# ftl/sdrainer

Measured on AMD Instinct MI355X. Metric: IQ MSamples/s through FFT+peak+envelope, higher is better.
Workload: dtype f64

## Files before the change

### sdrainer_amd/csrc/bank.h

```cpp
#pragma once
#include <hip/hip_runtime.h>

#include <algorithm>
#include <atomic>
#include <chrono>
#include <cmath>
#include <cstdio>
#include <cstdlib>
#include <cstring>
#include <memory>
#include <mutex>
#include <string>
#include <thread>
#include <vector>

#include "../../include/sdrainer_hip.h"
#include "host/delivery.h"
#include "host/frequency_mapping.h"
#include "sdr_device.h"

namespace sdrcapi {

inline thread_local std::string g_last_error;

// ... 72 lines not shown
    hipEvent_t done[sdr::K_COUNT] = {};
    void release()
    {
        psd.release();
        tap.release();
        tapw.release();
        tap_used.release();
        fft_ctr.release();
        fft_scratch.release();
        win_mean.release();
        cum_part.release();
        recs.release();
        raw_bits.release();
        bits.release();
        edges.release();
        edge_counts.release();
        tr_values.release();
        tr_raw.release();
        tr_deb.release();
        slots_before.release();
        cum_out.release();
        dev_peaks.release();
        peak_counts.release();
        for (auto &e : done) {
            if (e)
                (void)hipEventDestroy(e);
            e = nullptr;
        }
    }
};


enum Parts { PART_SPECTRA = 1, PART_LISTEN = 2, PART_ALL = 3 };

struct CursorPack {
    sdr::BatchCursor c[RING];
};

}

struct sdr_bank {
    template <class T>
    using DevBuf = sdrcapi::DevBuf<T>;
    using BatchSet = sdrcapi::BatchSet;
    static constexpr int N_STAGES = sdrcapi::N_STAGES, GRAPH_PHASES = sdrcapi::GRAPH_PHASES, N_GRAPHS = sdrcapi::N_GRAPHS, RING = sdrcapi::RING;

    sdr_config cfg{};
    sdr::Switches sw;
    int logn = 0;
    int hop = 0;
    int device = 0;
    hipStream_t stream[N_STAGES] = {};
    bool own_stream[N_STAGES] = {};

    int max_chunks = 0;
    int text_cap = 2048;
    int edge_cap = 0;
    int bit_words = 0;

    DevBuf<fft64::cplx> tw;
    DevBuf<unsigned char> db_tab;
    DevBuf<int32_t> tap_bins;
    DevBuf<float> window;
    bool windowed = false;
    DevBuf<float> spectrum_row;
    std::vector<BatchSet> set;
    DevBuf<sdr::BandState> band_state;
    DevBuf<sdr::ListenerSlot> slots;
    DevBuf<uint16_t> morse;
    DevBuf<uint32_t> text;
    DevBuf<uint32_t> text_frames;
    DevBuf<uint32_t> edge_pos;
    DevBuf<float> carry[2];

    std::vector<sdr::BandState> h_band_state;
    std::vector<sdr::ListenerSlot> h_slots;
    std::vector<int> n_slots;
    std::vector<int64_t> center_frequency;
    int carry_cur = 0;
    int cum_count = 0;
    int64_t total_frames = 0;
    int64_t batch_index = 0;
    int last_set = 0, last_frames = 0, last_chunks = 0, last_count0 = 0;
    int last_carry_in = 0;
    int edge_width = 0;
    int find_peaks = 1;
    bool failed = false;
    DevBuf<sdr::DropCounters> drops;
    DevBuf<sdr::BatchCursor> cursors;
    hipGraph_t graph[GRAPH_PHASES][N_GRAPHS] = {};
    hipGraphExec_t graph_exec[GRAPH_PHASES][N_GRAPHS] = {};
    hipGraphNode_t graph_cursor_node[GRAPH_PHASES] = {};
    hipEvent_t phase_done[GRAPH_PHASES][N_GRAPHS] = {};
    int64_t graph_base = 0;
    int64_t graph_replays = 0;
    bool graph_ready = false;
    int graph_frames = 0, graph_slots = 0;
    sdr::InFormat graph_fmt = sdr::InFormat::F32;
    uint64_t attach_gen = 0, graph_attach_gen = 0;
    bool graph_results_on = false;
    int graph_find_peaks = 0;
    bool defer_listen = false, listen_pending = false;
    struct PendingListen {
        int set = 0, frames = 0;
        int64_t first_frame = 0, batch = 0;
    } pend;
// ... 89 lines not shown
```

### sdrainer_amd/csrc/capi_bank.hip

```cpp
#include "bank.h"
#include "twiddles.h"

using namespace sdrcapi;

namespace sdr {
int set_error(int code, const char *msg) { return fail(code, msg); }
}

namespace sdrcapi {
std::unique_ptr<host::DeliveryBackend> make_results_backend(sdr_bank *b);

void resolve_profile(sdr_bank *b)
{
    for (auto &p : b->pending) {
        float ms = 0.f;
        if (hipEventElapsedTime(&ms, p.second.first, p.second.second) == hipSuccess) {
            b->prof_ms[p.first] += ms;
            b->prof_n[p.first] += 1;
        }
        (void)hipEventDestroy(p.second.first);
        (void)hipEventDestroy(p.second.second);
    }
    b->pending.clear();
}

int sync_bank(sdr_bank *b)
{
    HIP_TRY(hipSetDevice(b->device));
    {
        const int frc = flush_late_attached(b);
        if (frc)
            return frc;
    }
    for (int s = 0; s < N_STAGES; s++)
        HIP_TRY(hipStreamSynchronize(b->stream[s]));
    b->slots_put = false;
    resolve_profile(b);
    return SDR_OK;
}

int check_band(sdr_bank *b, int band)
{
    if (!b)
        return fail(SDR_ERR_BAD_ARG, "null bank");
    if (band < 0 || band >= b->cfg.n_bands)
        return fail(SDR_ERR_BAD_ARG, "band out of range");
    return SDR_OK;
}

int check_listener(sdr_bank *b, int band, int lid)
{
    int rc = check_band(b, band);
    if (rc)
        return rc;
    if (lid < 0 || lid >= b->n_slots[band])
        return fail(SDR_ERR_BAD_ARG, "listener id out of range");
    return SDR_OK;
}


hipError_t alloc_set(sdr_bank *b, BatchSet &S)
{
    const sdr_config &c = b->cfg;
    const size_t B = (size_t)c.n_bands, F = (size_t)c.max_batch_frames, L = (size_t)c.max_listeners, N = (size_t)c.block_size;
    hipError_t e = hipSuccess;
#define SET_ALLOC(buf, count)            \
    do {                                 \
        if (e == hipSuccess)             \
            e = (buf).alloc(count);      \
    } while (0)
    SET_ALLOC(S.psd, B * F * N);
    SET_ALLOC(S.tap, B * F * std::max<size_t>(L, 1));
    if (b->logn == 14) {
        SET_ALLOC(S.tapw, B * F * 4 * std::max<size_t>(L, 1));
        if (e == hipSuccess)
            e = S.tap_used.alloc(B * std::max<size_t>(L, 1), 0xff);
        SET_ALLOC(S.fft_ctr, B * 2);
    }
    SET_ALLOC(S.fft_scratch, B * (size_t)sdr::fft2p_group_frames(b->sw, c.block_size, c.n_bands, c.max_batch_frames) * N);
    SET_ALLOC(S.win_mean, B * F * 10);
    SET_ALLOC(S.recs, B * F);
    SET_ALLOC(S.raw_bits, B * L * (size_t)b->bit_words);
    SET_ALLOC(S.bits, B * L * (size_t)b->bit_words);
    SET_ALLOC(S.edges, B * L * (size_t)b->edge_cap);
    SET_ALLOC(S.edge_counts, B * L);
    if (c.trace) {
        SET_ALLOC(S.tr_values, B * F * L);
        SET_ALLOC(S.tr_raw, B * F * L);
        SET_ALLOC(S.tr_deb, B * F * L);
        SET_ALLOC(S.slots_before, B * L);
// ... 150 lines not shown
            return fail(SDR_ERR_HIP, "twiddle / table upload failed");
        }
    }
    b->res_backend = make_results_backend(b);
    b->results.reset(new host::Delivery(b->res_backend.get(), RING, GRAPH_PHASES * RING));
    b->set.reserve((size_t)RING + (size_t)GRAPH_PHASES * RING);
    b->set.resize(RING);
    for (int r = 0; r < RING; r++) {
        const hipError_t se = alloc_set(b, b->set[r]);
        if (se != hipSuccess) {
            sdr_destroy(b);
            return fail(SDR_ERR_HIP, std::string("allocating a batch buffer set: ") + hipGetErrorString(se));
        }
    }
    ALLOC(b->band_state, B);
    ALLOC(b->drops, 1);
    ALLOC(b->cursors, GRAPH_PHASES * RING);
    ALLOC(b->spectrum_row, (size_t)N);
    ALLOC(b->tap_bins, B * std::max<size_t>(L, 1));
    {
        std::vector<int32_t> free_bins(B * std::max<size_t>(L, 1), -1);
        hipError_t he = hipMemcpy(b->tap_bins.p, free_bins.data(), free_bins.size() * sizeof(int32_t), hipMemcpyHostToDevice);
        if (he != hipSuccess) {
            sdr_destroy(b);
            return fail(SDR_ERR_HIP, "tap table upload failed");
        }
    }
    ALLOC(b->slots, B * L);
    ALLOC(b->morse, cw::kMorseTableSize);
    ALLOC(b->text, B * L * (size_t)b->text_cap);
    ALLOC(b->text_frames, B * L * (size_t)b->text_cap);
    ALLOC(b->edge_pos, B * L * (size_t)cfg->max_batch_frames);
    ALLOC(b->carry[0], B * N);
    ALLOC(b->carry[1], B * N);
#undef ALLOC

    std::vector<uint16_t> h_morse(cw::kMorseTableSize);
    cw::build_morse_table(h_morse.data());
    hipError_t e = hipMemcpy(b->morse.p, h_morse.data(), sizeof(uint16_t) * cw::kMorseTableSize, hipMemcpyHostToDevice);
    b->h_band_state.assign(B, sdr::BandState{});
    for (auto &s : b->h_band_state)
        s.peak_threshold = cfg->peak_threshold;
    if (e == hipSuccess)
        e = hipMemcpy(b->band_state.p, b->h_band_state.data(), sizeof(sdr::BandState) * B, hipMemcpyHostToDevice);
    if (e != hipSuccess) {
        sdr_destroy(b);
        return fail(SDR_ERR_HIP, "state upload failed");
    }
    b->h_slots.assign(B * L, sdr::ListenerSlot{});
    b->n_slots.assign(B, 0);
    b->center_frequency.assign(B, 0);
    b->staged.assign(B, sdr::StreamStage{N, b->hop, 0, 0});
    b->staged_kind.assign(B, 0);
    *out = b;
    return SDR_OK;
}

int sdr_destroy(sdr_bank *b)
{
    if (!b)
        return SDR_OK;
    (void)hipSetDevice(b->device);
    for (int s = 0; s < N_STAGES; s++)
        (void)hipStreamSynchronize(b->stream[s]);
    resolve_profile(b);
    drop_graphs(b);
    if (b->slots_put_ev)
        (void)hipEventDestroy(b->slots_put_ev);
    for (auto &ph : b->phase_done)
        for (auto &ev : ph)
            if (ev)
                (void)hipEventDestroy(ev);
    b->tw.release();
    b->drops.release();
    b->cursors.release();
    b->db_tab.release();
    b->tap_bins.release();
    b->window.release();
    b->spectrum_row.release();
    for (auto &S : b->set)
        S.release();
    if (b->results)
        for (int i = 0; i < b->results->n_sets(); i++) {
            host::ResultSet &rs = b->results->set(i);
            if (rs.block)
                (void)hipHostFree(rs.block);
            if (rs.ev_listen)
                (void)hipEventDestroy(static_cast<hipEvent_t>(rs.ev_listen));
            if (rs.ev_peaks)
                (void)hipEventDestroy(static_cast<hipEvent_t>(rs.ev_peaks));
        }
    b->band_state.release();
    b->slots.release();
    b->morse.release();
    b->text.release();
    b->text_frames.release();
    b->edge_pos.release();
    b->carry[0].release();
    b->carry[1].release();
    for (int s = 0; s < N_STAGES; s++)
        if (b->own_stream[s] && b->stream[s])
            (void)hipStreamDestroy(b->stream[s]);
    if (b->copy_stream) {
        (void)hipStreamSynchronize(b->copy_stream);
        (void)hipStreamDestroy(b->copy_stream);
    }
    for (auto &st : b->stage) {
        if (st.h_f32)
            (void)hipHostFree(st.h_f32);
        if (st.h_raw)
            (void)hipHostFree(st.h_raw);
        st.d_f32.release();
        st.d_raw.release();
        if (st.uploaded)
            (void)hipEventDestroy(st.uploaded);
        if (st.consumed)
            (void)hipEventDestroy(st.consumed);
    }
    delete b;
    return SDR_OK;
}

int sdr_set_stream(sdr_bank *b, void *hip_stream)
{
    if (!b)
        return fail(SDR_ERR_BAD_ARG, "null bank");
    int rc = sync_bank(b);
    if (rc)
        return rc;
    for (int s = 1; s < N_STAGES; s++)
        if (!b->own_stream[s])
            b->stream[s] = reinterpret_cast<hipStream_t>(hip_stream);
    b->stream[S_FFT] = reinterpret_cast<hipStream_t>(hip_stream);
    return SDR_OK;
}

int sdr_sync(sdr_bank *b)
{
    if (!b)
        return fail(SDR_ERR_BAD_ARG, "null bank");
    return sync_bank(b);
}

int sdr_attach(sdr_bank *b, int band, int bin, int *listener_id)
{
    int rc = check_band(b, band);
    if (rc)
        return rc;
    const sdr_config &c = b->cfg;
    if (bin < 0 || bin >= c.block_size)
        return fail(SDR_ERR_BAD_ARG, "bin out of range");
    int lid = -1;
    for (int i = 0; i < b->n_slots[band]; i++)
        if (!b->h_slots[(size_t)band * c.max_listeners + i].active) {
            lid = i;
            break;
        }
    if (lid < 0) {
        if (b->n_slots[band] >= c.max_listeners)
            return fail(SDR_ERR_NO_SLOT, "listener pool exhausted");
        lid = b->n_slots[band]++;
    }
    sdr::ListenerSlot &s = b->h_slots[(size_t)band * c.max_listeners + lid];
    memset(&s, 0, sizeof s);
    s.active = 1;
    s.bin = bin;
    cw::debouncer_init(s.deb, c.signal_debounce);
    cw::decoder_init(s.dec, c.sample_rate, sdr::effective_hop(c.hop, c.block_size));
    cw::decoder_reset(s.dec);
    s.start_frame = s.tapped_from = (uint32_t)b->total_frames;
    rc = sync_bank(b);
    if (rc)
        return rc;
    HIP_TRY(hipMemcpy(b->slots.p + (size_t)band * c.max_listeners + lid, &s, sizeof s, hipMemcpyHostToDevice));
    const int32_t tap_bin = bin;
    HIP_TRY(hipMemcpy(b->tap_bins.p + (size_t)band * c.max_listeners + lid, &tap_bin, sizeof tap_bin, hipMemcpyHostToDevice));
    b->attach_gen++;
    if (listener_id)
        *listener_id = lid;
    return SDR_OK;
}

int sdr_detach(sdr_bank *b, int band, int lid)
{
    int rc = check_listener(b, band, lid);
    if (rc)
        return rc;
// ... 209 lines not shown
```

### sdrainer_amd/csrc/capi_process.hip

```cpp
#include <string>

#include "bank.h"

using namespace sdrcapi;

namespace sdrcapi {

constexpr int PUT_SLOTS = 16, PUT_BINS = 128;
struct SlotPack {
    int32_t n;
    int32_t index[PUT_SLOTS];
    sdr::ListenerSlot slot[PUT_SLOTS];
};
struct BinPack {
    int32_t n;
    int32_t index[PUT_BINS], bin[PUT_BINS];
};
__global__ void k_put_slots(sdr::ListenerSlot *slots, SlotPack p)
{
    constexpr int W = sizeof(sdr::ListenerSlot) / 4;
    static_assert(sizeof(sdr::ListenerSlot) % 4 == 0, "word copy");
    for (int i = threadIdx.x; i < p.n * W; i += blockDim.x)
        reinterpret_cast<uint32_t *>(slots + p.index[i / W])[i % W] = reinterpret_cast<const uint32_t *>(&p.slot[i / W])[i % W];
}
// ... 33 lines not shown
        HIP_TRY(hipGetLastError());
    }
    b->late_attached.clear();
    return SDR_OK;
}


int process_device_impl(sdr_bank *b, const void *iq_dev, int n_frames, size_t in_stride, sdr::InFormat fmt)
{
    if (b->failed)
        return fail(SDR_ERR_STATE, "an earlier process call failed half way; destroy the bank");
    if (b->graph_ready)
        return fail(SDR_ERR_STATE, "a graph is captured: process through sdr_graph_launch, or sdr_graph_release first");
    if (b->listen_pending)
        return fail(SDR_ERR_STATE, "the previous batch still waits for its listen half (sdr_process_listen)");
    const int rc = process_device_body(b, iq_dev, n_frames, in_stride, -1, -1, b->defer_listen ? PART_SPECTRA : PART_ALL, fmt);
    if (rc == SDR_ERR_HIP)
        b->failed = true;
    return rc;
}

int process_device_body(sdr_bank *b, const void *iq_dev, int n_frames, size_t in_stride, int capture_k, int capture_stage, int parts,
                        sdr::InFormat fmt)
{
    const bool cap = capture_k >= 0;
    const bool do_spectra = (parts & PART_SPECTRA) != 0, do_listen = (parts & PART_LISTEN) != 0;
    if (!do_spectra)
        n_frames = b->pend.frames;
    const sdr::BatchCursor *cur = cap ? b->cursors.p + capture_k : nullptr;
    const sdr_config &c = b->cfg;
    if (n_frames <= 0)
        return SDR_OK;
    struct DisarmOnExit {
        ~DisarmOnExit() { sdr::t_done_event = nullptr; }
    } disarm_on_exit;
    if (n_frames > c.max_batch_frames)
        return fail(SDR_ERR_BAD_ARG, "n_frames exceeds max_batch_frames");
    HIP_TRY(hipSetDevice(b->device));
    if (!cap) {
        const int frc = flush_late_attached(b);
        if (frc)
            return frc;
    }
    const int B = c.n_bands, N = c.block_size, stride = c.max_batch_frames;
    const sdr::NoiseGeom ng = b->noise_geom();
    const int si = cap ? RING + capture_k : do_spectra ? (int)(b->batch_index % RING) : b->pend.set;
    const int64_t first_frame = do_spectra ? b->total_frames : b->pend.first_frame;
    BatchSet &S = b->set[si];
    host::ResultSet &RS = b->results->set(si);
    int max_slots = 0;
    for (int i = 0; i < B; i++)
        max_slots = std::max(max_slots, b->n_slots[i]);
    const int count0 = b->cum_count;
    const sdr::BatchPlan P = sdr::plan_batch(b->sw, sdr::BatchGeometry{B, N, stride, b->max_chunks}, n_frames, count0, cap, max_slots, b->windowed);
    const int *plan = P.stream;
    const sdr::CumGeom cg{N, stride, n_frames, count0, b->max_chunks};
#define SDR_ON(k) (!cap || (capture_stage == G_THRESHOLDS ? (k) == sdr::K_THRESHOLDS : (plan[k] == capture_stage && (k) != sdr::K_THRESHOLDS)))
#if defined(SDR_DIAG)
#define SDR_LAUNCH(id, call) \
    do {                     \
        if (!(b->sw.diag_skip >> (id) & 1) && SDR_ON(id)) \
            HIP_TRY(call);   \
    } while (0)
#else
#define SDR_LAUNCH(id, call)  \
    do {                      \
        if (SDR_ON(id))       \
            HIP_TRY(call);    \
    } while (0)
#endif
    auto stream_of = [&](int k) { return b->stream[plan[k]]; };
    auto after = [&](int k, int dep) -> int {
        if (stream_of(k) != stream_of(dep) && !cap)
            HIP_TRY(hipStreamWaitEvent(stream_of(k), S.done[dep], 0));
        return SDR_OK;
    };
#define SDR_AFTER(k, dep)          \
    do {                           \
        int _rc = after((k), (dep)); \
        if (_rc)                   \
            return _rc;            \
    } while (0)
#define SDR_ARM(k) (sdr::t_done_event = cap ? nullptr : S.done[k])
#define SDR_DONE(k)                                                                                   \
    do {                                                                                              \
        if (sdr::t_done_event && !cap) {                                                              \
            sdr::t_done_event = nullptr;                                                              \
            HIP_TRY(hipEventRecord(S.done[k], stream_of(k)));                                         \
        }                                                                                             \
    } while (0)

    if (do_spectra) {
    if (b->results_on && !cap) {
        const int prc = b->results->park(si);
        if (prc)
            return prc;
    }
    {
        static const int launch_order[] = {sdr::K_WINDOW_MEANS, sdr::K_NOISE_STATS, sdr::K_THRESHOLDS, sdr::K_LISTEN_GATHER,
                                           sdr::K_LISTEN_DECODE, sdr::K_CUMULATE,   sdr::K_FIND_PEAKS};
        int last_on[N_STAGES];
        for (int &l : last_on)
            l = -1;
        for (int k : launch_order)
            last_on[plan[k]] = k;
        for (int st = 0; st < N_STAGES; st++) {
            const int k = last_on[st];
// ... 478 lines not shown
```

### sdrainer_amd/csrc/host/batch_plan.h

```cpp
#pragma once
#include <cstdint>
#include <cstdlib>
#include <cstring>

#include "../../../include/sdrainer_hip.h"

namespace sdr {

enum KernelId {
    K_FFT = 0, K_WINDOW_MEANS, K_NOISE_STATS, K_THRESHOLDS, K_LISTEN_GATHER, K_CUMULATE, K_FIND_PEAKS, K_LISTEN_DECODE,
    K_COUNT
};
enum Stage { S_FFT = 0, S_NOISE, S_LISTEN, S_PEAKS, N_STAGES };

constexpr int kR32MaxTap = 512;

struct Switches {
    bool noise_scan = true;
    int force_exact = 0;
    int fft_r32 = -1;
    int fft_fpw = 0;
    int cum_bound = -1;
    int refine_wide = -1;
    int var_mfma = -1;
    int wm_wpb = 0;
    int fft2p_group_mb = -1;
    bool no_overlap = false;
    bool graph_debug = false;
    int diag_skip = 0;
    int diag_plan[K_COUNT] = {-1, -1, -1, -1, -1, -1, -1, -1};
};

inline int tri_state(const char *e)
{
    if (!e)
        return -1;
    const int v = atoi(e);
    return v >= 0 ? (v != 0 ? 1 : 0) : -1;
}

inline Switches read_switches()
{
    Switches s;
    const char *e;
    if ((e = getenv("SDR_NOISE_PATH")))
        s.noise_scan = strcmp(e, "chains") != 0;
    if ((e = getenv("SDR_NOISE_FORCE_EXACT")))
        s.force_exact = atoi(e);
    if ((e = getenv("SDR_FFT_R32")))
        s.fft_r32 = atoi(e) ? 1 : 0;
    if ((e = getenv("SDR_FFT_FPW"))) {
        const int v = atoi(e);
        s.fft_fpw = v < 1 ? 1 : (v > 64 ? 64 : v);
    }
    s.cum_bound = tri_state(getenv("SDR_CUM_BOUND"));
    s.refine_wide = tri_state(getenv("SDR_REFINE_WIDE"));
    s.var_mfma = tri_state(getenv("SDR_VAR_MFMA"));
    if ((e = getenv("SDR_FFT2P_GROUP_MB")))
        s.fft2p_group_mb = atoi(e) >= 0 ? atoi(e) : -1;
    if ((e = getenv("SDR_WM_WPB")))
        s.wm_wpb = atoi(e) > 0 ? atoi(e) : 0;
    e = getenv("SDR_NO_OVERLAP");
    s.no_overlap = e && e[0] == '1';
    s.graph_debug = getenv("SDR_GRAPH_DEBUG") != nullptr;
#if defined(SDR_DIAG)
    if ((e = getenv("SDR_DIAG_SKIP")))
        s.diag_skip = atoi(e);
    if ((e = getenv("SDR_DIAG_PLAN")))
        for (int k = 0; k < K_COUNT && e[k] >= '0' && e[k] < '0' + N_STAGES; k++)
            s.diag_plan[k] = e[k] - '0';
#endif
    return s;
}

inline bool noise_scan_at(const Switches &sw, int n) { return sw.noise_scan && n <= 16384; }
inline bool var_mfma_at(const Switches &sw, int n, int n_frames)
{
    if (sw.var_mfma >= 0)
        return sw.var_mfma != 0;
    return n <= 16384 && n_frames < 4096;
}
inline bool may_use_matrix_pipe(const Switches &sw, int n) { return !noise_scan_at(sw, n) && (sw.var_mfma == 1 || (sw.var_mfma < 0 && n <= 16384)); }

struct FftChoice {
    bool r32 = false;
    int fpw = 0;
    bool wide_tap = false;
    bool two_phase = false;
    int group_frames = 0;
};

constexpr int kFft2pGroupMiB = 128;
inline int fft2p_group_frames(const Switches &sw, int n, int n_bands, int max_frames)
{
    if (n <= 16384 || n_bands <= 0 || max_frames <= 0)
        return 0;
    const int mib = sw.fft2p_group_mb >= 0 ? sw.fft2p_group_mb : kFft2pGroupMiB;
    const long per_frame = (long)n_bands * n * 16;
    const long f = mib == 0 ? max_frames : ((long)mib << 20) / per_frame;
    return (int)(f < 1 ? 1 : (f > max_frames ? max_frames : f));
}

inline FftChoice fft_choice(const Switches &sw, int n, int n_frames, int n_bands, int tap_n, bool windowed = false)
{
    FftChoice c;
    c.r32 = !windowed && n == 16384 && tap_n <= kR32MaxTap && (sw.fft_r32 == 1 || (sw.fft_r32 < 0 && (long)n_frames * n_bands >= 1024));
    c.fpw = sw.fft_fpw;
    c.wide_tap = c.r32 && tap_n > 0;
    c.two_phase = n > 16384;
    return c;
}

enum class Refine { NONE, NARROW, WIDE };

struct BatchGeometry {
    int n_bands, n, max_batch_frames, max_chunks;
};

struct BatchPlan {
    int stream[K_COUNT];
    FftChoice fft;
    bool noise_scan;
    int force_exact;
    bool var_mfma;
    int wm_wpb;
    bool bound;
    bool bound_done;
    int scan_parts;
    int n_slots;
    int n_chunks;
    int new_count;
    Refine refine;
};

inline BatchPlan plan_batch(const Switches &sw, const BatchGeometry &g, int n_frames, int count0, bool capturing, int max_slots,
                            bool windowed = false)
{
    BatchPlan p;
    const int plan[K_COUNT] = { S_FFT,         S_NOISE,  S_NOISE,  S_PEAKS,
                                S_LISTEN,   S_PEAKS,      S_PEAKS,   S_LISTEN};
    for (int k = 0; k < K_COUNT; k++)
        p.stream[k] = plan[k];
    if (!capturing && (long)g.n_bands * g.n <= 8192)
        p.stream[K_LISTEN_GATHER] = S_PEAKS;
    for (int k = 0; k < K_COUNT; k++)
        if (sw.diag_plan[k] >= 0)
            p.stream[k] = sw.diag_plan[k];

    p.fft = fft_choice(sw, g.n, n_frames, g.n_bands, max_slots, windowed);
    p.fft.group_frames = fft2p_group_frames(sw, g.n, g.n_bands, g.max_batch_frames);

    p.noise_scan = noise_scan_at(sw, g.n);
    p.force_exact = sw.force_exact;
    p.var_mfma = var_mfma_at(sw, g.n, n_frames);
    p.wm_wpb = sw.wm_wpb;

    p.bound = sw.cum_bound >= 0 ? sw.cum_bound != 0 : (double)n_frames * (double)g.n_bands * (double)g.n >= 64.0 * 1024.0 * 1024.0;
    p.bound_done = p.noise_scan && p.bound;

    p.n_chunks = (count0 + n_frames) / SDR_CUMULATION_SIZE;
    p.new_count = (count0 + n_frames) % SDR_CUMULATION_SIZE;
    p.n_slots = p.n_chunks + (p.new_count != 0 ? 1 : 0);
    if (capturing) {
        p.n_chunks = (SDR_CUMULATION_SIZE - 1 + n_frames) / SDR_CUMULATION_SIZE;
        p.n_slots = p.n_chunks + 1;
    }
    p.scan_parts = (long)p.n_slots * g.n_bands < 64 ? 2 : 1;

    const bool wide = sw.refine_wide >= 0 ? sw.refine_wide != 0 : (g.n >= 4096 && (long)p.n_chunks * g.n_bands >= 64);
    p.refine = !p.bound ? Refine::NONE : wide ? Refine::WIDE : Refine::NARROW;
    return p;
}

}
```

### sdrainer_amd/csrc/k_fft_psd.hip

```cpp
#include <hip/hip_runtime.h>

#include <algorithm>
#include <cstdlib>
#include <mutex>

#include "../../include/sdrainer_hip.h"
#include "cw_decoder.h"
#include "fft_f64.h"
#include "fft_r32.h"
#include "gomath.h"
#include "sc16.h"
#include "sdr_device.h"

#if !defined(SDR_FFT_WIN)
#define SDR_FFT_WIN 0
#endif
#if SDR_FFT_WIN
#define SDR_K_FFT_PSD k_fft_psd_win
#define SDR_K_FFT_PSD_SC16 k_fft_psd_sc16_win
#define SDR_WIN_PARAM , const float *__restrict__ win
#define SDR_WIN_ARG , win
#else
#define SDR_K_FFT_PSD k_fft_psd
#define SDR_K_FFT_PSD_SC16 k_fft_psd_sc16
// ... 896 lines not shown
        return hipGetLastError();
    }
    int fpw = fpw_asked > 0 ? fpw_asked : kDefaultFpw;
    while (fpw > 1 && (long)((n_frames + fpw - 1) / fpw) * n_bands < 256)
        fpw /= 2;
    if (fpw > 1)
        launch_kernel((SDR_K_FFT_PSD<LOGN, true>), dim3((n_frames + fpw - 1) / fpw, n_bands), dim3(PL::T), fft64::kLdsBytes<LOGN>, stream,
                           iq, cur, tw, psd, in_stride, frame_stride, out_stride, n_frames, fpw, tap.bins, tap.out, tap.n, tap.stride SDR_WIN_ARG);
    else
        launch_kernel((SDR_K_FFT_PSD<LOGN, false>), dim3(n_frames, n_bands), dim3(PL::T),
                           fft64::kLdsBytes<LOGN> + tap_lds + kPfSinkBytes, stream, iq, cur, tw, psd, in_stride,
                           frame_stride, out_stride, n_frames, 1, tap.bins, tap.out, tap.n, tap.stride SDR_WIN_ARG);
    return hipGetLastError();
    }
}

#if SDR_FFT_WIN
void window_layout(int logn, const float *w, float *out)
{
    switch (logn) {
    case 9: window_layout_t<9>(w, out); break;
    case 10: window_layout_t<10>(w, out); break;
    case 11: window_layout_t<11>(w, out); break;
    case 12: window_layout_t<12>(w, out); break;
    case 13: window_layout_t<13>(w, out); break;
    case 14: window_layout_t<14>(w, out); break;
    default:
        for (int i = 0; i < 1 << logn; i++)
            out[i] = w[i];
        break;
    }
}

hipError_t launch_fft_win(int logn, FftChoice fft, InFormat fmt, const void *iq, const BatchCursor *cur, const fft64::cplx *tw, float *psd,
                          int n_frames, int n_bands, size_t in_stride, int frame_stride, int out_stride, FftTap tap, hipStream_t stream)
{
    if (!tap.window || fft.r32 || fft.two_phase)
        return hipErrorInvalidValue;
#else
hipError_t launch_fft(int logn, FftChoice fft, InFormat fmt, const void *iq, const BatchCursor *cur, const fft64::cplx *tw, float *psd,
                      int n_frames, int n_bands, size_t in_stride, int frame_stride, int out_stride, FftTap tap, hipStream_t stream)
{
    if (fmt != InFormat::F32 && fmt != InFormat::SC16)
        return hipErrorInvalidValue;
    if (fft.two_phase)
        return launch_fft_2p(logn, fft, fmt, iq, cur, tw, psd, n_frames, n_bands, in_stride, frame_stride, out_stride, tap, stream);
    if (tap.window)
        return launch_fft_win(logn, fft, fmt, iq, cur, tw, psd, n_frames, n_bands, in_stride, frame_stride, out_stride, tap, stream);
    if (fft.r32) {
        if (logn != 14)
            return hipErrorInvalidValue;
        const fft64::cplx *tw32 = tw + fft64::Plan<14>::TW_TOTAL;
        if (fmt == InFormat::SC16)
            return launch_fft_r32_sc16(static_cast<const int16_t *>(iq), cur, tw32, psd, n_frames, n_bands, in_stride, frame_stride, out_stride, tap, stream);
        return launch_fft_r32(static_cast<const float *>(iq), cur, tw32, psd, n_frames, n_bands, in_stride, frame_stride, out_stride, tap, stream);
    }
#endif
    switch (logn) {
    case 9: return launch_fft_t<9>(fft.fpw, fmt, iq, cur, tw, psd, n_frames, n_bands, in_stride, frame_stride, out_stride, tap, stream);
    case 10: return launch_fft_t<10>(fft.fpw, fmt, iq, cur, tw, psd, n_frames, n_bands, in_stride, frame_stride, out_stride, tap, stream);
    case 11: return launch_fft_t<11>(fft.fpw, fmt, iq, cur, tw, psd, n_frames, n_bands, in_stride, frame_stride, out_stride, tap, stream);
    case 12: return launch_fft_t<12>(fft.fpw, fmt, iq, cur, tw, psd, n_frames, n_bands, in_stride, frame_stride, out_stride, tap, stream);
    case 13: return launch_fft_t<13>(fft.fpw, fmt, iq, cur, tw, psd, n_frames, n_bands, in_stride, frame_stride, out_stride, tap, stream);
    case 14: return launch_fft_t<14>(fft.fpw, fmt, iq, cur, tw, psd, n_frames, n_bands, in_stride, frame_stride, out_stride, tap, stream);
    default: return hipErrorInvalidValue;
    }
}
#if !SDR_FFT_WIN
hipError_t launch_fft(int logn, FftChoice fft, const float *iq, const BatchCursor *cur, const fft64::cplx *tw, float *psd, int n_frames,
                      int n_bands, size_t in_stride, int frame_stride, int out_stride, FftTap tap, hipStream_t stream)
{
    return launch_fft(logn, fft, InFormat::F32, iq, cur, tw, psd, n_frames, n_bands, in_stride, frame_stride, out_stride, tap, stream);
}

int twiddle_count(int logn)
{
    switch (logn) {
    case 9: return fft64::Plan<9>::TW_TOTAL;
    case 10: return fft64::Plan<10>::TW_TOTAL;
    case 11: return fft64::Plan<11>::TW_TOTAL;
    case 12: return fft64::Plan<12>::TW_TOTAL;
    case 13: return fft64::Plan<13>::TW_TOTAL;
    case 14: return fft64::Plan<14>::TW_TOTAL + r32_twiddle_count();
    case 15: return 1 << 14;
    case 16: return 1 << 15;
    default: return 0;
    }
}

void build_twiddles(int logn, const double *wre, const double *wim, fft64::cplx *out)
{
    switch (logn) {
    case 9: fft64::build_pass_twiddles<9>(wre, wim, out); break;
    case 10: fft64::build_pass_twiddles<10>(wre, wim, out); break;
    case 11: fft64::build_pass_twiddles<11>(wre, wim, out); break;
    case 12: fft64::build_pass_twiddles<12>(wre, wim, out); break;
    case 13: fft64::build_pass_twiddles<13>(wre, wim, out); break;
    case 14:
        fft64::build_pass_twiddles<14>(wre, wim, out);
        r32_build_twiddles(wre, wim, out + fft64::Plan<14>::TW_TOTAL);
        break;
    case 15:
    case 16:
        for (int i = 0; i < 1 << (logn - 1); i++)
            out[i] = fft64::cplx{wre[i], wim[i]};
        break;
    default: break;
    }
// ... 5 lines not shown
```

### sdrainer_amd/csrc/k_fft_r32.hip

```cpp
#include <hip/hip_runtime.h>

#include <algorithm>
#include <mutex>

#include "fft_r32.h"
#include "sdr_device.h"

#if !defined(SDR_R32_SC16)
#define SDR_R32_SC16 0
#endif
#if !defined(SDR_R32_HOP)
#define SDR_R32_HOP 0
#endif
#if SDR_R32_SC16
#include "sc16.h"
#define SDR_R32_IN int16_t
#else
#define SDR_R32_IN float
#endif
#if SDR_R32_HOP && SDR_R32_SC16
#define SDR_R32_KERNEL k_fft_r32_hop_sc16
#define SDR_R32_LAUNCH launch_fft_r32_hop_sc16
#elif SDR_R32_HOP
#define SDR_R32_KERNEL k_fft_r32_hop
// ... 437 lines not shown
        __syncthreads();
        SDR_R32_STAMP(st, RS_ROW);
        pf_point(PF_ROW);
        {
#pragma unroll
            for (int j = 0; j < N / 4 / T; j++)
                sv[j] = *reinterpret_cast<const u32x4 *>(smem + row_word(4 * (t + T * j)) * 4);
            const float *row = reinterpret_cast<const float *>(smem);
            const float tv = row[row_word(my_bin & (N - 1))];
            tapv = my_bin >= 0 ? tv : 0.0f;
            if (__builtin_amdgcn_readfirstlane(t) < n_tap && wide_b) {
                const rsrc_t wr = make_rsrc(wide_b + (size_t)frame * (4 * tap_stride), reg_tap ? (unsigned)tap_stride * 16u : 0u);
                u32x4 wv;
                wv.x = __float_as_uint(row[row_word((my_bin - 1) & (N - 1))]);
                wv.y = __float_as_uint(tv);
                wv.z = __float_as_uint(row[row_word((my_bin + 1) & (N - 1))]);
                wv.w = 0u;
                __builtin_amdgcn_raw_buffer_store_b128(wv, wr, t < n_tap ? (unsigned)t * 16u : 0x7ffffff0u, 0, 0);
            }
        }
        const unsigned after = __builtin_amdgcn_readfirstlane(claim_lds[0]);
        soft_arrive(soft + SOFT_ROW);
        SDR_R32_STAMP(st, RS_STORED);
#if defined(SDR_R32_PHASES)
        if (st.on && (threadIdx.x & 63) < RS_COUNT)
            g_r32_phases[threadIdx.x >> 6][threadIdx.x & 63] = st.v;
#endif
        prev = frame;
        frame = next;
        next = after;
        it++;
    }
    int t = tid;
    asm volatile("" : "+v"(t));
    flush_row(prev, t, 0, N / 4 / T);
    if (t == 0) {
        unsigned *const ctr = band_ctr();
        const unsigned done = __hip_atomic_fetch_add(ctr + 1, 1u, __ATOMIC_ACQ_REL, __HIP_MEMORY_SCOPE_AGENT);
        if (done == stash[2] - 1) {
            __hip_atomic_store(ctr, 0u, __ATOMIC_RELAXED, __HIP_MEMORY_SCOPE_AGENT);
            __hip_atomic_store(ctr + 1, 0u, __ATOMIC_RELAXED, __HIP_MEMORY_SCOPE_AGENT);
        }
    }
#endif
}

}

#if !SDR_R32_SC16 && !SDR_R32_HOP
int r32_twiddle_count() { return fft32::kTwTotal; }
void r32_build_twiddles(const double *wre, const double *wim, fft64::cplx *out) { fft32::build_twiddles(wre, wim, out); }
#endif

#if !defined(SDR_R32_RESERVE)
#define SDR_R32_RESERVE 0
#endif

hipError_t SDR_R32_LAUNCH(const SDR_R32_IN *iq, const BatchCursor *cur, const fft64::cplx *tw, float *psd, int n_frames, int n_bands,
                          size_t in_stride, int frame_stride, int out_stride, FftTap tap, hipStream_t stream)
{
    constexpr int kMaxDevices = 64;
    static std::once_flag setup_once[kMaxDevices];
    static hipError_t setup_err[kMaxDevices];
    static int cu_count[kMaxDevices];
    int dev = 0;
    hipError_t e = hipGetDevice(&dev);
    if (e != hipSuccess)
        return e;
    if (dev < 0 || dev >= kMaxDevices)
        return hipErrorInvalidDevice;
    std::call_once(setup_once[dev], [dev] {
        hipError_t se = hipFuncSetAttribute(reinterpret_cast<const void *>(&r32::SDR_R32_KERNEL), hipFuncAttributeMaxDynamicSharedMemorySize,
                                            r32::kLdsBytes);
        if (se == hipSuccess)
            se = hipDeviceGetAttribute(&cu_count[dev], hipDeviceAttributeMultiprocessorCount, dev);
        setup_err[dev] = se;
    });
    if (setup_err[dev] != hipSuccess)
        return setup_err[dev];
    if (n_frames <= 0 || n_bands <= 0)
        return hipSuccess;
    if (tap.n > fft32::T)
        return hipErrorInvalidValue;
    if (!tap.steal)
        return hipErrorInvalidValue;
    if (in_stride > 0xffffffffu)
        return hipErrorInvalidValue;
#if SDR_R32_HOP
    int shift = 0;
    while ((1 << shift) < frame_stride)
        shift++;
    if (frame_stride <= 0 || (1 << shift) != frame_stride || n_frames >= (1 << r32::kFrameBits))
        return hipErrorInvalidValue;
    const unsigned frames_and_shift = (unsigned)n_frames | (unsigned)shift << r32::kFrameBits;
#else
    if (frame_stride != fft32::N)
#if SDR_R32_SC16
        return launch_fft_r32_hop_sc16(iq, cur, tw, psd, n_frames, n_bands, in_stride, frame_stride, out_stride, tap, stream);
#else
        return launch_fft_r32_hop(iq, cur, tw, psd, n_frames, n_bands, in_stride, frame_stride, out_stride, tap, stream);
#endif
    const unsigned frames_and_shift = (unsigned)n_frames;
#endif
    const int cus = std::max(1, cu_count[dev] - SDR_R32_RESERVE);
    const int grid = std::min((cus + n_bands - 1) / n_bands, n_frames);
    launch_kernel(r32::SDR_R32_KERNEL, dim3(grid, n_bands), dim3(fft32::T), r32::kLdsBytes, stream, iq, cur, tw, psd, (unsigned)in_stride, out_stride,
                  frames_and_shift, tap.steal, tap.bins, tap.out, tap.n, tap.stride, tap.wide, tap.used);
    return hipGetLastError();
}

}
```

### sdrainer_amd/csrc/sdr_device.h

```cpp
#pragma once
#include <hip/hip_ext.h>
#include <hip/hip_runtime.h>

#include <cstdint>
#include <initializer_list>
#include <mutex>

#include "../../include/sdrainer_hip.h"
#include "cw_decoder.h"
#include "fft_f64.h"
#include "host/batch_plan.h"
#include "host/overlap.h"

namespace sdr {

struct BandState {
    float nf_ring[SDR_NOISE_WINDOW];
    float dev_ring[SDR_NOISE_WINDOW];
    float nf_sum, dev_sum;
    int32_t next;
    float peak_threshold;
};

struct ListenerSlot {
// ... 73 lines not shown
    if (done)
        hipExtLaunchKernelGGL(kernel, grid, block, lds_bytes, stream, nullptr, done, 0, args...);
    else
        hipLaunchKernelGGL(kernel, grid, block, lds_bytes, stream, args...);
}

struct LdsLimitOnce {
    static constexpr int kMaxDevices = 64;
    std::once_flag dev[kMaxDevices];
};
inline hipError_t raise_lds_limit_once(LdsLimitOnce &once, std::initializer_list<const void *> kernels, int bytes)
{
    int dev = 0;
    hipError_t e = hipGetDevice(&dev);
    if (e != hipSuccess)
        return e;
    if (dev < 0 || dev >= LdsLimitOnce::kMaxDevices)
        return hipErrorInvalidDevice;
    hipError_t attr_err = hipSuccess;
    std::call_once(once.dev[dev], [&] {
        for (const void *k : kernels) {
            const hipError_t ae = hipFuncSetAttribute(k, hipFuncAttributeMaxDynamicSharedMemorySize, bytes);
            if (ae != hipSuccess)
                attr_err = ae;
        }
    });
    return attr_err;
}

struct FftTap {
    const int32_t *bins;
    float *out;
    int n;
    int stride;
    float *wide = nullptr;
    int32_t *used = nullptr;
    uint32_t *steal = nullptr;
    fft64::cplx *scratch = nullptr;
    const float *window = nullptr;
};

hipError_t launch_fft(int logn, FftChoice fft, InFormat fmt, const void *iq, const BatchCursor *cur, const fft64::cplx *tw, float *psd,
                      int n_frames, int n_bands, size_t in_stride, int frame_stride, int out_stride, FftTap tap, hipStream_t stream);
hipError_t launch_fft(int logn, FftChoice fft, const float *iq, const BatchCursor *cur, const fft64::cplx *tw, float *psd, int n_frames,
                      int n_bands, size_t in_stride, int frame_stride, int out_stride, FftTap tap, hipStream_t stream);
hipError_t launch_fft_win(int logn, FftChoice fft, InFormat fmt, const void *iq, const BatchCursor *cur, const fft64::cplx *tw, float *psd,
                          int n_frames, int n_bands, size_t in_stride, int frame_stride, int out_stride, FftTap tap, hipStream_t stream);
void window_layout(int logn, const float *w, float *out);
hipError_t launch_fft_2p(int logn, FftChoice fft, InFormat fmt, const void *iq, const BatchCursor *cur, const fft64::cplx *tw, float *psd,
                         int n_frames, int n_bands, size_t in_stride, int frame_stride, int out_stride, FftTap tap, hipStream_t stream);
int twiddle_count(int logn);
void build_twiddles(int logn, const double *wre, const double *wim, fft64::cplx *out);
hipError_t launch_fft_r32(const float *iq, const BatchCursor *cur, const fft64::cplx *tw, float *psd, int n_frames, int n_bands,
                          size_t in_stride, int frame_stride, int out_stride, FftTap tap, hipStream_t stream);
hipError_t launch_fft_r32_sc16(const int16_t *iq, const BatchCursor *cur, const fft64::cplx *tw, float *psd, int n_frames, int n_bands,
                               size_t in_stride, int frame_stride, int out_stride, FftTap tap, hipStream_t stream);
hipError_t launch_fft_r32_hop(const float *iq, const BatchCursor *cur, const fft64::cplx *tw, float *psd, int n_frames, int n_bands,
                              size_t in_stride, int frame_stride, int out_stride, FftTap tap, hipStream_t stream);
hipError_t launch_fft_r32_hop_sc16(const int16_t *iq, const BatchCursor *cur, const fft64::cplx *tw, float *psd, int n_frames, int n_bands,
                                   size_t in_stride, int frame_stride, int out_stride, FftTap tap, hipStream_t stream);
int r32_twiddle_count();
void r32_build_twiddles(const double *wre, const double *wim, fft64::cplx *out);
hipError_t launch_window_means(const float *psd, double *win_mean, NoiseGeom g, int n_frames, int n_bands, int stride, int wpb_forced,
                               hipStream_t stream);
hipError_t launch_noise_stats(const float *psd, const double *win_mean, sdr_frame_rec *recs, NoiseGeom g, int n_frames,
                              int n_bands, int stride, bool mfma, hipStream_t stream);
hipError_t launch_mfma_order_probe(unsigned *mismatches, int order, hipStream_t stream);
hipError_t launch_thresholds(sdr_frame_rec *recs, BandState *st, int n_frames, int n_bands, int stride,
                             hipStream_t stream);
hipError_t launch_listen_gather(const float *tap, const float *psd, const sdr_frame_rec *recs, const ListenerSlot *slots, const void *db_tab,
                                uint64_t *raw_bits, float *tr_values, uint8_t *tr_raw, const BatchCursor *cur, ListenGeom g, int n_frames,
                                int n_slots, int n_bands, hipStream_t stream);
hipError_t launch_listen_decode(ListenerSlot *slots, const uint16_t *morse, const uint64_t *raw_bits,
                                uint64_t *deb_bits, uint32_t *text, uint32_t *text_frames, sdr_edge *edges,
                                uint32_t *edge_counts, uint8_t *tr_deb, DropCounters *drops, const BatchCursor *cur, ListenGeom g,
                                int n_frames, int n_bands, uint32_t *edge_pos, int pos_stride, hipStream_t stream);
hipError_t launch_listener_stop(ListenerSlot *slot, const uint16_t *morse, uint32_t *text, uint32_t *text_frames, int text_cap,
                                uint32_t frame, DropCounters *drops, hipStream_t stream);
hipError_t launch_set_debounce(ListenerSlot *slots, int n, int threshold, hipStream_t stream);
hipError_t launch_cumulate(const float *psd, const void *db_tab, float *carry0, float *carry1, int carry_in, float *cum_out,
                           const float *cum_part, const BatchCursor *cur, CumGeom g, int n_slots, int n_bands, bool bound, bool bound_done,
                           int parts, hipStream_t stream);
hipError_t launch_psd_scan(const float *psd, sdr_frame_rec *recs, float *cum_out, float *cum_part, const BatchCursor *cur, NoiseGeom ng,
                           CumGeom cg, int n_slots, int n_bands, bool do_bound, int parts, int force_exact, hipStream_t stream);
hipError_t launch_noise_exact_check(const float *psd_band, sdr_frame_rec *recs_band, NoiseGeom ng, int n_frames, unsigned *mismatches,
                                    hipStream_t stream);
hipError_t launch_spectrum_row(const float *psd_row, float *out, int n, hipStream_t stream);
hipError_t launch_pack_listen(ListenerSlot *slots, const sdr_edge *edges, const uint32_t *edge_counts, const uint32_t *text,
                              const uint32_t *text_frames, const DropCounters *drops, ResultsLayout lay, int n_slots, int n_bands, unsigned char *host,
                              hipStream_t stream);
hipError_t launch_pack_peaks(const DevPeak *peaks, const int *counts, const BatchCursor *cur, ResultsLayout lay, int find_peaks,
                             int n_frames, int n_chunks, int n_bands, unsigned char *host, hipStream_t stream);
__host__ __device__ inline int chunks_completed(int count0, int n_frames)
{
    const int first_len = SDR_CUMULATION_SIZE - count0;
    return n_frames >= first_len ? 1 + (n_frames - first_len) / SDR_CUMULATION_SIZE : 0;
}
hipError_t launch_unpack_be16(const uint8_t *raw, float *out, size_t n_values, hipStream_t stream);
hipError_t launch_unpack_sc16(const int16_t *raw, float *out, size_t n_values, hipStream_t stream);
hipError_t launch_find_peaks(float *cum, const float *psd, const void *db_tab, const float *carry0, const float *carry1, int carry_in,
                             const sdr_frame_rec *recs, DevPeak *peaks, int *counts, const BatchCursor *cur, PeakGeom g, int n_frames,
                             int n_chunks, int n_bands, Refine refine, FftTap tap, hipStream_t stream);
hipError_t launch_cumulation_row(const float *psd_band, const void *db_tab, const float *carry_in_band, float *row_out, CumGeom g, int slot,
                                 hipStream_t stream);

}
```

Before: 198,700.

## Reserve CUs for overlapping noise scan by capping r32 FFT grid size

```diff
diff --git a/sdrainer_amd/csrc/bank.h b/sdrainer_amd/csrc/bank.h
--- a/sdrainer_amd/csrc/bank.h
+++ b/sdrainer_amd/csrc/bank.h
@@ -148,6 +148,7 @@
     int device = 0;
     hipStream_t stream[N_STAGES] = {};
     bool own_stream[N_STAGES] = {};
+    bool fft_queue_alone = true;
 
     int max_chunks = 0;
     int text_cap = 2048;
diff --git a/sdrainer_amd/csrc/capi_bank.hip b/sdrainer_amd/csrc/capi_bank.hip
--- a/sdrainer_amd/csrc/capi_bank.hip
+++ b/sdrainer_amd/csrc/capi_bank.hip
@@ -36,6 +36,68 @@
         HIP_TRY(hipStreamSynchronize(b->stream[s]));
     b->slots_put = false;
     resolve_profile(b);
+    return SDR_OK;
+}
+
+constexpr int kProbeSpinUs = 300;
+__global__ void k_queue_probe_spin(unsigned ticks, unsigned *sink)
+{
+    const unsigned long long t0 = wall_clock64();
+    unsigned n = 0;
+    for (int i = 0; i < (1 << 20) && wall_clock64() - t0 < ticks; i++) {
+        __builtin_amdgcn_s_sleep(32);
+        n++;
+    }
+    if (n == 0xffffffffu)
+        *sink = n;
+}
+__global__ void k_queue_probe_nop() {}
+
+int probe_fft_queue(sdr_bank *b)
+{
+    b->fft_queue_alone = true;
+    if (b->cfg.block_size != 16384 || b->sw.no_overlap || b->sw.fft_reserve >= 0)
+        return SDR_OK;
+    HIP_TRY(hipSetDevice(b->device));
+    hipEvent_t spin_done = nullptr, nop_done[N_STAGES] = {};
+    auto cleanup = [&] {
+        if (spin_done)
+            (void)hipEventDestroy(spin_done);
+        for (hipEvent_t e : nop_done)
+            if (e)
+                (void)hipEventDestroy(e);
+    };
+    hipError_t e = hipEventCreateWithFlags(&spin_done, hipEventDisableTiming);
+    for (int s = 1; s < N_STAGES && e == hipSuccess; s++)
+        e = hipEventCreateWithFlags(&nop_done[s], hipEventDisableTiming);
+    for (int s = 0; s < N_STAGES && e == hipSuccess; s++) {
+        hipLaunchKernelGGL(k_queue_probe_nop, dim3(1), dim3(1), 0, b->stream[s]);
+        e = hipStreamSynchronize(b->stream[s]);
+    }
+    if (e == hipSuccess) {
+        hipLaunchKernelGGL(k_queue_probe_spin, dim3(1), dim3(1), 0, b->stream[S_FFT], (unsigned)kProbeSpinUs * 100u, reinterpret_cast<unsigned *>(b->drops.p));
+        e = hipEventRecord(spin_done, b->stream[S_FFT]);
+    }
+    for (int s = 1; s < N_STAGES && e == hipSuccess; s++) {
+        hipLaunchKernelGGL(k_queue_probe_nop, dim3(1), dim3(1), 0, b->stream[s]);
+        e = hipEventRecord(nop_done[s], b->stream[s]);
+    }
+    bool shared[N_STAGES] = {};
+    for (int s = 1; s < N_STAGES && e == hipSuccess; s++) {
+        e = hipEventSynchronize(nop_done[s]);
+        shared[s] = b->stream[s] == b->stream[S_FFT] || hipEventQuery(spin_done) == hipSuccess;
+        if (shared[s])
+            b->fft_queue_alone = false;
+    }
+    if (e == hipSuccess)
+        e = hipStreamSynchronize(b->stream[S_FFT]);
+    cleanup();
+    if (e != hipSuccess)
+        return fail(SDR_ERR_HIP, std::string("hardware queue probe: ") + hipGetErrorString(e));
+    if (b->sw.queue_debug)
+        fprintf(stderr, "sdr: FFT stream %s (noise %d listen %d peaks %d share its hardware queue)\n",
+                b->fft_queue_alone ? "has a hardware queue to itself" : "SHARES a hardware queue: no CUs reserved", (int)shared[S_NOISE], (int)shared[S_LISTEN],
+                (int)shared[S_PEAKS]);
     return SDR_OK;
 }
 
@@ -292,6 +354,13 @@
     b->center_frequency.assign(B, 0);
     b->staged.assign(B, sdr::StreamStage{N, b->hop, 0, 0});
     b->staged_kind.assign(B, 0);
+    {
+        const int prc = probe_fft_queue(b);
+        if (prc) {
+            sdr_destroy(b);
+            return prc;
+        }
+    }
     *out = b;
     return SDR_OK;
 }
@@ -372,7 +441,7 @@
         if (!b->own_stream[s])
             b->stream[s] = reinterpret_cast<hipStream_t>(hip_stream);
     b->stream[S_FFT] = reinterpret_cast<hipStream_t>(hip_stream);
-    return SDR_OK;
+    return probe_fft_queue(b);
 }
 
 int sdr_sync(sdr_bank *b)
diff --git a/sdrainer_amd/csrc/capi_process.hip b/sdrainer_amd/csrc/capi_process.hip
--- a/sdrainer_amd/csrc/capi_process.hip
+++ b/sdrainer_amd/csrc/capi_process.hip
@@ -109,7 +109,7 @@
     for (int i = 0; i < B; i++)
         max_slots = std::max(max_slots, b->n_slots[i]);
     const int count0 = b->cum_count;
-    const sdr::BatchPlan P = sdr::plan_batch(b->sw, sdr::BatchGeometry{B, N, stride, b->max_chunks}, n_frames, count0, cap, max_slots, b->windowed);
+    const sdr::BatchPlan P = sdr::plan_batch(b->sw, sdr::BatchGeometry{B, N, stride, b->max_chunks, b->fft_queue_alone}, n_frames, count0, cap, max_slots, b->windowed);
     const int *plan = P.stream;
     const sdr::CumGeom cg{N, stride, n_frames, count0, b->max_chunks};
 #define SDR_ON(k) (!cap || (capture_stage == G_THRESHOLDS ? (k) == sdr::K_THRESHOLDS : (plan[k] == capture_stage && (k) != sdr::K_THRESHOLDS)))
diff --git a/sdrainer_amd/csrc/host/batch_plan.h b/sdrainer_amd/csrc/host/batch_plan.h
--- a/sdrainer_amd/csrc/host/batch_plan.h
+++ b/sdrainer_amd/csrc/host/batch_plan.h
@@ -22,11 +22,13 @@
     int fft_fpw = 0;
     int cum_bound = -1;
     int refine_wide = -1;
+    int fft_reserve = -1;
     int var_mfma = -1;
     int wm_wpb = 0;
     int fft2p_group_mb = -1;
     bool no_overlap = false;
     bool graph_debug = false;
+    bool queue_debug = false;
     int diag_skip = 0;
     int diag_plan[K_COUNT] = {-1, -1, -1, -1, -1, -1, -1, -1};
 };
@@ -56,6 +58,8 @@
     s.cum_bound = tri_state(getenv("SDR_CUM_BOUND"));
     s.refine_wide = tri_state(getenv("SDR_REFINE_WIDE"));
     s.var_mfma = tri_state(getenv("SDR_VAR_MFMA"));
+    if ((e = getenv("SDR_FFT_RESERVE")))
+        s.fft_reserve = atoi(e) >= 0 ? atoi(e) : -1;
     if ((e = getenv("SDR_FFT2P_GROUP_MB")))
         s.fft2p_group_mb = atoi(e) >= 0 ? atoi(e) : -1;
     if ((e = getenv("SDR_WM_WPB")))
@@ -63,6 +67,7 @@
     e = getenv("SDR_NO_OVERLAP");
     s.no_overlap = e && e[0] == '1';
     s.graph_debug = getenv("SDR_GRAPH_DEBUG") != nullptr;
+    s.queue_debug = getenv("SDR_QUEUE_DEBUG") != nullptr;
 #if defined(SDR_DIAG)
     if ((e = getenv("SDR_DIAG_SKIP")))
         s.diag_skip = atoi(e);
@@ -88,6 +93,8 @@
     bool wide_tap = false;
     bool two_phase = false;
     int group_frames = 0;
+    int reserve_cus = 0;
+    bool reserve_forced = false;
 };
 
 constexpr int kFft2pGroupMiB = 128;
@@ -111,10 +118,28 @@
     return c;
 }
 
+constexpr int kReserveRounds = 2;
+constexpr int kReserveExtra = 24;
+constexpr int kReserveMax = 64;
+constexpr int kReserveDeviceShare = 4;
+constexpr int kReserveMinFrames = 2048;
+inline int fft_reserve_cus(const Switches &sw, const FftChoice &c, bool noise_scan, int n_frames, int n_bands, int scan_wgs, bool fft_queue_alone = true)
+{
+    if (!c.r32)
+        return 0;
+    if (sw.fft_reserve >= 0)
+        return sw.fft_reserve;
+    if (!noise_scan || !fft_queue_alone || (long)n_frames * n_bands < kReserveMinFrames)
+        return 0;
+    const int r = (scan_wgs + kReserveRounds - 1) / kReserveRounds + kReserveExtra;
+    return r > kReserveMax ? kReserveMax : r;
+}
+
 enum class Refine { NONE, NARROW, WIDE };
 
 struct BatchGeometry {
     int n_bands, n, max_batch_frames, max_chunks;
+    bool fft_queue_alone = true;
 };
 
 struct BatchPlan {
@@ -166,6 +191,8 @@
         p.n_slots = p.n_chunks + 1;
     }
     p.scan_parts = (long)p.n_slots * g.n_bands < 64 ? 2 : 1;
+    p.fft.reserve_cus = fft_reserve_cus(sw, p.fft, p.noise_scan, n_frames, g.n_bands, p.n_slots * p.scan_parts * g.n_bands, g.fft_queue_alone);
+    p.fft.reserve_forced = p.fft.r32 && sw.fft_reserve >= 0;
 
     const bool wide = sw.refine_wide >= 0 ? sw.refine_wide != 0 : (g.n >= 4096 && (long)p.n_chunks * g.n_bands >= 64);
     p.refine = !p.bound ? Refine::NONE : wide ? Refine::WIDE : Refine::NARROW;
diff --git a/sdrainer_amd/csrc/k_fft_psd.hip b/sdrainer_amd/csrc/k_fft_psd.hip
--- a/sdrainer_amd/csrc/k_fft_psd.hip
+++ b/sdrainer_amd/csrc/k_fft_psd.hip
@@ -972,8 +972,8 @@
             return hipErrorInvalidValue;
         const fft64::cplx *tw32 = tw + fft64::Plan<14>::TW_TOTAL;
         if (fmt == InFormat::SC16)
-            return launch_fft_r32_sc16(static_cast<const int16_t *>(iq), cur, tw32, psd, n_frames, n_bands, in_stride, frame_stride, out_stride, tap, stream);
-        return launch_fft_r32(static_cast<const float *>(iq), cur, tw32, psd, n_frames, n_bands, in_stride, frame_stride, out_stride, tap, stream);
+            return launch_fft_r32_sc16(static_cast<const int16_t *>(iq), cur, tw32, psd, n_frames, n_bands, in_stride, frame_stride, out_stride, tap, fft.reserve_cus, fft.reserve_forced, stream);
+        return launch_fft_r32(static_cast<const float *>(iq), cur, tw32, psd, n_frames, n_bands, in_stride, frame_stride, out_stride, tap, fft.reserve_cus, fft.reserve_forced, stream);
     }
 #endif
     switch (logn) {
diff --git a/sdrainer_amd/csrc/k_fft_r32.hip b/sdrainer_amd/csrc/k_fft_r32.hip
--- a/sdrainer_amd/csrc/k_fft_r32.hip
+++ b/sdrainer_amd/csrc/k_fft_r32.hip
@@ -513,12 +513,8 @@
 void r32_build_twiddles(const double *wre, const double *wim, fft64::cplx *out) { fft32::build_twiddles(wre, wim, out); }
 #endif
 
-#if !defined(SDR_R32_RESERVE)
-#define SDR_R32_RESERVE 0
-#endif
-
 hipError_t SDR_R32_LAUNCH(const SDR_R32_IN *iq, const BatchCursor *cur, const fft64::cplx *tw, float *psd, int n_frames, int n_bands,
-                          size_t in_stride, int frame_stride, int out_stride, FftTap tap, hipStream_t stream)
+                          size_t in_stride, int frame_stride, int out_stride, FftTap tap, int reserve_cus, bool reserve_forced, hipStream_t stream)
 {
     constexpr int kMaxDevices = 64;
     static std::once_flag setup_once[kMaxDevices];
@@ -557,13 +553,14 @@
 #else
     if (frame_stride != fft32::N)
 #if SDR_R32_SC16
-        return launch_fft_r32_hop_sc16(iq, cur, tw, psd, n_frames, n_bands, in_stride, frame_stride, out_stride, tap, stream);
-#else
-        return launch_fft_r32_hop(iq, cur, tw, psd, n_frames, n_bands, in_stride, frame_stride, out_stride, tap, stream);
+        return launch_fft_r32_hop_sc16(iq, cur, tw, psd, n_frames, n_bands, in_stride, frame_stride, out_stride, tap, reserve_cus, reserve_forced, stream);
+#else
+        return launch_fft_r32_hop(iq, cur, tw, psd, n_frames, n_bands, in_stride, frame_stride, out_stride, tap, reserve_cus, reserve_forced, stream);
 #endif
     const unsigned frames_and_shift = (unsigned)n_frames;
 #endif
-    const int cus = std::max(1, cu_count[dev] - SDR_R32_RESERVE);
+    const int reserve = reserve_forced ? reserve_cus : std::min(reserve_cus, cu_count[dev] / kReserveDeviceShare);
+    const int cus = std::max(1, cu_count[dev] - std::max(0, reserve));
     const int grid = std::min((cus + n_bands - 1) / n_bands, n_frames);
     launch_kernel(r32::SDR_R32_KERNEL, dim3(grid, n_bands), dim3(fft32::T), r32::kLdsBytes, stream, iq, cur, tw, psd, (unsigned)in_stride, out_stride,
                   frames_and_shift, tap.steal, tap.bins, tap.out, tap.n, tap.stride, tap.wide, tap.used);
diff --git a/sdrainer_amd/csrc/sdr_device.h b/sdrainer_amd/csrc/sdr_device.h
--- a/sdrainer_amd/csrc/sdr_device.h
+++ b/sdrainer_amd/csrc/sdr_device.h
@@ -149,13 +149,13 @@
 int twiddle_count(int logn);
 void build_twiddles(int logn, const double *wre, const double *wim, fft64::cplx *out);
 hipError_t launch_fft_r32(const float *iq, const BatchCursor *cur, const fft64::cplx *tw, float *psd, int n_frames, int n_bands,
-                          size_t in_stride, int frame_stride, int out_stride, FftTap tap, hipStream_t stream);
+                          size_t in_stride, int frame_stride, int out_stride, FftTap tap, int reserve_cus, bool reserve_forced, hipStream_t stream);
 hipError_t launch_fft_r32_sc16(const int16_t *iq, const BatchCursor *cur, const fft64::cplx *tw, float *psd, int n_frames, int n_bands,
-                               size_t in_stride, int frame_stride, int out_stride, FftTap tap, hipStream_t stream);
+                               size_t in_stride, int frame_stride, int out_stride, FftTap tap, int reserve_cus, bool reserve_forced, hipStream_t stream);
 hipError_t launch_fft_r32_hop(const float *iq, const BatchCursor *cur, const fft64::cplx *tw, float *psd, int n_frames, int n_bands,
-                              size_t in_stride, int frame_stride, int out_stride, FftTap tap, hipStream_t stream);
+                              size_t in_stride, int frame_stride, int out_stride, FftTap tap, int reserve_cus, bool reserve_forced, hipStream_t stream);
 hipError_t launch_fft_r32_hop_sc16(const int16_t *iq, const BatchCursor *cur, const fft64::cplx *tw, float *psd, int n_frames, int n_bands,
-                                   size_t in_stride, int frame_stride, int out_stride, FftTap tap, hipStream_t stream);
+                                   size_t in_stride, int frame_stride, int out_stride, FftTap tap, int reserve_cus, bool reserve_forced, hipStream_t stream);
 int r32_twiddle_count();
 void r32_build_twiddles(const double *wre, const double *wim, fft64::cplx *out);
 hipError_t launch_window_means(const float *psd, double *win_mean, NoiseGeom g, int n_frames, int n_bands, int stride, int wpb_forced,
```

Result: faster. 215,800, median of 6 (+8.6%).
